# boqian-li/GarmentDreamer

Hardware: AMD Instinct MI355X
Metric: SDS iters/sec (rasterize+UNet+bwd), 100k Gaussians ×8 views @512², 1/2/4/8 GPU (higher is better)
Workload: dtype bf16

## Files before the change

### garmentdreamer_amd/csrc/nn_conv3x3.hip

```cpp
#include <hip/hip_runtime.h>
#include <stdlib.h>
#include <stdint.h>
#include <stdio.h>

#include <mutex>
#include <vector>

#include "../../include/gd_nn.h"
#include "nn_device.h"
#include "nn_host.h"

#ifndef GD_CONV_ABLATE
#define GD_CONV_ABLATE 0
#endif

namespace {

using namespace gdnn;

#ifndef GD_PATCH_EPI
#define GD_PATCH_EPI 0
#endif
typedef __attribute__((ext_vector_type(4))) float f32x4;

constexpr int BK = 64;

struct ConvGeom {
    int Hin, Win, Hg, Wg, sy, sx, Hout, Wout, osy, osx, ooy, oox, ntaps, back;
    int wtaps;
    uint64_t ty4, tx4, w4;
};

template <int BN, int BM, int WN, int WM>
__device__ __forceinline__ void conv3x3_nhwc_bf16_body(
    const uint16_t* __restrict__ in, const uint16_t* __restrict__ wt, const uint16_t* __restrict__ bias,
    int bias_img_stride, const uint16_t* __restrict__ residual, uint16_t* __restrict__ out, int Nimg, const ConvGeom& g,
    int Cin, int Cout, int tiles_n, int nwg, float* __restrict__ partial, int steps_per_split, int bid_raw, int split_idx)
{
// ... 1085 lines not shown
        g_cprof.total_flops += flops;
        g_cprof.total_bytes += bytes;
        a = b = nullptr;
    }
    ~ProfScope()
    {
        if (!a && !b) return;
        std::lock_guard<std::mutex> lk(g_cprof.mu);
        if (a) g_cprof.pool.push_back(a);
        if (b) g_cprof.pool.push_back(b);
    }
    void close_s1(int64_t M, int Cin, int Cout, bool residual)
    {
        close(2.0 * (double)M * Cout * 9.0 * Cin,
              2.0 * ((double)M * Cin + 9.0 * Cin * Cout + (double)M * Cout + (residual ? (double)M * Cout : 0.0)));
    }
};

struct TiledArgs {
    void* stream;
    const void* x;
    const float* mean_rstd;
    const void *gamma, *beta;
    int groups, silu;
    const void *w, *bias;
    int bias_img_stride;
    const void* residual;
    void* y;
    int N, H, W, Cin, Cout;
    float* stat_part;
};
constexpr int kCuLds = 160 * 1024;
static bool gn_table_fits(int lds, int Cin) { return lds + gn_table_bytes(Cin) <= kCuLds; }
template <auto Kern>
int launch_tiled(const TiledArgs& a, int lds, int tile_w, int bn, bool persistent)
{
    const int dev = current_device();
    if (dev < 0) return dev;
    if (a.mean_rstd) {
        if (!gn_table_fits(lds, a.Cin)) return fail(GD_NN_ERR_INVALID_ARG, "GroupNorm scale / shift table of Cin channels does not fit the LDS");
        lds += gn_table_bytes(a.Cin);
    }
    if (const int r = reserve_lds<Kern>(dev, a.mean_rstd ? kCuLds : lds)) return r;
    hipStream_t s = (hipStream_t)a.stream;
    const int tiles_x = (a.W + tile_w - 1) / tile_w, tiles_y = (a.H + 15) / 16, tiles_n = (a.Cout + bn - 1) / bn;
    const int nwg = a.N * tiles_x * tiles_y * tiles_n;
    int grid = nwg;
    if (persistent && nwg > num_cus(dev)) grid = (nwg & 7) == 0 ? (num_cus(dev) & ~7) : num_cus(dev);
    ProfScope prof(s);
    hipLaunchKernelGGL(Kern, dim3(grid), dim3(512), lds, s, (const uint16_t*)a.x, (const uint16_t*)a.w,
                       (const uint16_t*)a.bias, a.bias_img_stride, (const uint16_t*)a.residual, (uint16_t*)a.y, a.N, a.H,
                       a.W, a.Cin, a.Cout, a.mean_rstd, (const uint16_t*)a.gamma, (const uint16_t*)a.beta, a.groups, a.silu,
                       tiles_n, tiles_x, tiles_y, nwg, a.stat_part);
    prof.close_s1((int64_t)a.N * a.H * a.W, a.Cin, a.Cout, a.residual != nullptr);
    return launch_status();
}

}

extern "C" {

const char* gd_nn_conv_last_error(void) { return g_err; }

static int pick_split(int64_t tiles, int steps, int target = 420)
{
    int s = (int)((target + tiles / 2) / tiles);
    const int cap = steps * 2 / 15 < 24 ? steps * 2 / 15 : 24;
    if (s > cap) s = cap;
    return s < 2 ? 1 : s;
}

static size_t split_ws_bytes(int split, int64_t M, int Cout)
{
    return (size_t)split * (size_t)((M + 255) / 256 * 2) * (size_t)((Cout + 127) / 128) * 16384u * sizeof(float);
}

static int split_tile_px(int64_t M, int Cout)
{
    const int forced = conv_env().split_px;
    if (forced == 128 || forced == 256) return forced;
    M *= g_route_scale;
    return (M >= 1024 && Cout >= 1024) || M >= 2048 ? 256 : 128;
}

static bool small_tile_nosplit(int64_t M, int Cout, int ntaps, int Cin)
{
// ... 289 lines not shown
    return (size_t)((Cout + 127) / 128) * 3 * (size_t)(Cin / kWinoCK) * (size_t)kWinoWStage;
}

int gd_nn_conv3x3_wino_weights(void* stream, const void* weight, void* u, int Cout, int Cin)
{
    if (!weight || !u || Cout <= 0 || Cin <= 0) return fail(GD_NN_ERR_INVALID_ARG, "wino_weights: bad argument");
    if (Cin % kWinoCK) return fail(GD_NN_ERR_INVALID_ARG, "wino_weights: Cin % 32 != 0");
    const size_t total = gd_nn_conv3x3_wino_weights_bytes(Cout, Cin) / 16;
    const int grid = (int)((total + 255) / 256 < 4096 ? (total + 255) / 256 : 4096);
    hipLaunchKernelGGL(conv3x3_wino_weights_kernel, dim3(grid), dim3(256), 0, (hipStream_t)stream, (const uint16_t*)weight,
                       (uint16_t*)u, Cout, Cin);
    return launch_status();
}

int gd_nn_conv3x3_wino_supported(int N, int H, int W, int Cin, int Cout)
{
    if (N <= 0 || H < 16 || W < 16 || Cin <= 0 || Cout < 64) return 0;
    if (Cin % kWinoCK || Cout % 8) return 0;
    if ((double)N * H * W * Cin * 2.0 >= 2147483648.0 || (double)gd_nn_conv3x3_wino_weights_bytes(Cout, Cin) >= 2147483648.0) return 0;
    return 1;
}

static int launch_wino(void* stream, const void* x, const float* mean_rstd, const void* gamma, const void* beta, int groups,
                       int apply_silu, const void* u, const void* bias, int bias_img_stride, const void* residual, void* y,
                       int N, int H, int W, int Cin, int Cout, float* stat_part)
{
    if (!x || !u || !y) return fail(GD_NN_ERR_INVALID_ARG, "null pointer");
    if (!gd_nn_conv3x3_wino_supported(N, H, W, Cin, Cout))
        return fail(GD_NN_ERR_INVALID_ARG, "conv3x3_wino: need Cin % 32 == 0, Cout % 8 == 0, Cout >= 64, H, W >= 16, tensors < 2 GiB");
    if (mean_rstd && (!gamma || !beta || groups <= 0 || Cin % groups))
        return fail(GD_NN_ERR_INVALID_ARG, "conv3x3_wino: GroupNorm needs gamma, beta and Cin % groups == 0");
    const TiledArgs a = {stream, x, mean_rstd, gamma, beta, groups, apply_silu, u, bias, bias_img_stride, residual, y,
                         N, H, W, Cin, Cout, stat_part};
    return mean_rstd ? launch_tiled<conv3x3_wino_kernel<true>>(a, kWinoLds, 16, 128, false)
                     : launch_tiled<conv3x3_wino_kernel<false>>(a, kWinoLds, 16, 128, false);
}

int gd_nn_conv3x3_wino_forward(void* stream, const void* x, const void* u, const void* bias, int bias_img_stride,
                               const void* residual, void* y, int N, int H, int W, int Cin, int Cout, float* stat_part)
{
    return launch_wino(stream, x, nullptr, nullptr, nullptr, 0, 0, u, bias, bias_img_stride, residual, y, N, H, W, Cin,
                       Cout, stat_part);
}

int gd_nn_conv3x3_wino_gn_forward(void* stream, const void* x, const float* mean_rstd, const void* gamma, const void* beta,
                                  int groups, int apply_silu, const void* u, const void* bias, int bias_img_stride,
                                  const void* residual, void* y, int N, int H, int W, int Cin, int Cout, float* stat_part)
{
    if (!mean_rstd) return fail(GD_NN_ERR_INVALID_ARG, "conv3x3_wino_gn: mean_rstd is NULL");
    return launch_wino(stream, x, mean_rstd, gamma, beta, groups, apply_silu, u, bias, bias_img_stride, residual, y, N, H, W,
                       Cin, Cout, stat_part);
}

size_t gd_nn_conv3x3_wide_weights_bytes(int Cout, int Cin)
{
    if (Cout <= 0 || Cin <= 0 || Cin % kWideCK) return 0;
    return (size_t)((Cout + 127) / 128) * 3 * (size_t)(Cin / kWideCK) * (size_t)kWideWStage;
}

int gd_nn_conv3x3_wide_weights(void* stream, const void* weight, void* u, int Cout, int Cin)
{
    if (!weight || !u || Cout <= 0 || Cin <= 0 || Cin % kWideCK) return fail(GD_NN_ERR_INVALID_ARG, "wide_weights: bad argument");
    const size_t total = gd_nn_conv3x3_wide_weights_bytes(Cout, Cin) / 16;
    const int grid = (int)((total + 255) / 256 < 4096 ? (total + 255) / 256 : 4096);
    hipLaunchKernelGGL(conv3x3_wide_weights_kernel, dim3(grid), dim3(256), 0, (hipStream_t)stream, (const uint16_t*)weight,
                       (uint16_t*)u, Cout, Cin);
    return launch_status();
}

// ... 349 lines not shown
```

### garmentdreamer_amd/csrc/nn_conv_wino.h

```cpp
#pragma once
#include "nn_device.h"

#ifndef GD_WINO_ABLATE
#define GD_WINO_ABLATE 0
#endif

constexpr int kWinoCK = 32;
constexpr int kWinoVStage = 4 * 18 * 8 * kWinoCK * 2;
constexpr int kWinoWStage = 4 * 128 * kWinoCK * 2;
constexpr int kWinoPBytes = 21 * 1024;
constexpr int kWinoLds = 2 * kWinoVStage + 2 * kWinoWStage + kWinoPBytes;

__device__ __forceinline__ uint16_t f2bf_finite(float f)
{
    uint32_t u = __float_as_uint(f);
    u += 0x7fffu + ((u >> 16) & 1u);
    return (uint16_t)(u >> 16);
}

__global__ __launch_bounds__(256) void conv3x3_wino_weights_kernel(const uint16_t* __restrict__ w,
                                                                   uint16_t* __restrict__ u, int Cout, int Cin)
{
    const int kc = Cin / kWinoCK;
    const int tiles_n = (Cout + 127) / 128;
    const size_t total = (size_t)tiles_n * 3 * kc * 2048;
    for (size_t i = (size_t)blockIdx.x * blockDim.x + threadIdx.x; i < total; i += (size_t)gridDim.x * blockDim.x) {
        const int q = (int)(i & 2047);
        const size_t sl = i >> 11;
        const int c = (int)(sl % kc);
        const int ky = (int)((sl / kc) % 3);
        const int tn = (int)(sl / kc / 3);
        const int pc = q & 3, row = (q >> 2) & 127, pos = q >> 9;
        const int co = tn * 128 + row;
        const int ci0 = c * kWinoCK + ((pc ^ ((row >> 2) & 3)) << 3);
        uint16_t o[8];
#pragma unroll
        for (int e = 0; e < 8; e++) {
            uint16_t v = 0;
            if (co < Cout) {
                const uint16_t* g = w + ((size_t)co * 3 + ky) * 3 * Cin + ci0 + e;
                const float g0 = bf2f(g[0]), g1 = bf2f(g[Cin]), g2 = bf2f(g[2 * Cin]);
                v = pos == 0 ? g[0] : pos == 3 ? g[2 * Cin]
                    : pos == 1 ? f2bf_finite(0.5f * ((g0 + g2) + g1)) : f2bf_finite(0.5f * ((g0 + g2) - g1));
            }
            o[e] = v;
        }
        *(uint4*)(u + i * 8) = *(const uint4*)o;
    }
}

template <bool GN>
__global__ __launch_bounds__(512) void conv3x3_wino_kernel(
    const uint16_t* __restrict__ in, const uint16_t* __restrict__ uw, const uint16_t* __restrict__ bias,
    int bias_img_stride, const uint16_t* __restrict__ residual, uint16_t* __restrict__ out, int Nimg, int H, int W,
    int Cin, int Cout, const float* __restrict__ mean_rstd, const uint16_t* __restrict__ gamma,
    const uint16_t* __restrict__ beta, int G, int apply_silu, int tiles_n, int tiles_x, int tiles_y, int nwg,
    float* __restrict__ stat_part)
{
    constexpr int BN = 128;
    constexpr int THREADS = 512;
    typedef __attribute__((ext_vector_type(4))) uint32_t u32x4;
    extern __shared__ __attribute__((aligned(16))) char smem[];
    char* sV = smem;
    char* sW = smem + 2 * kWinoVStage;
    char* sP = smem + 2 * kWinoVStage + 2 * kWinoWStage;

    const int tid = threadIdx.x, lane = tid & 63;
    const int wave = __builtin_amdgcn_readfirstlane(tid >> 6);
    int bid = blockIdx.x;
    if ((nwg & 7) == 0) bid = (bid & 7) * (nwg >> 3) + (bid >> 3);
    const int tn = bid % tiles_n, tm = bid / tiles_n;
    const int tpi = tiles_x * tiles_y;
    const int nimg = tm / tpi, trem = tm - nimg * tpi;
    const int tyi = trem / tiles_x, txi = trem - tyi * tiles_x;
    const int y0 = tyi * 16 - 1, x0 = txi * 16 - 1;
    const int n0 = tn * BN;

    const uint32_t row_bytes = (uint32_t)Cin * 2u;
    const __amdgpu_buffer_rsrc_t rs_in = buffer_rsrc(in, (uint32_t)Nimg * (uint32_t)(H * W) * row_bytes);
    const int kc = Cin / kWinoCK;
    const __amdgpu_buffer_rsrc_t rs_w = buffer_rsrc(uw, (uint32_t)tiles_n * 3u * (uint32_t)kc * (uint32_t)kWinoWStage);

    uint32_t p_goff[3];
    uint32_t p_keep = 0;
#pragma unroll
    for (int i = 0; i < 3; i++) {
        const int q = tid + THREADS * i;
        const int pix = q >> 2;
        const int py = pix / kPatch, px = pix - py * kPatch;
        const int gy = y0 + py, gx = x0 + px;
        const bool inimg = pix < kPatchPix && (unsigned)gy < (unsigned)H && (unsigned)gx < (unsigned)W;
        p_goff[i] = inimg ? (uint32_t)((nimg * H + gy) * W + gx) * row_bytes + (uint32_t)(q & 3) * 16u : kOOB;
        if (inimg) p_keep |= 1u << i;
    }
    auto issueP = [&](int c) {
        if (GD_WINO_ABLATE == 3) return;
#pragma unroll
        for (int i = 0; i < 3; i++) {
            if (i == 2 && wave >= 5) continue;
            bload_lds16(rs_in, p_goff[i], (uint32_t)c * (kWinoCK * 2), sP + (wave * 64 + THREADS * i) * 16);
        }
    };
    u32x4 p_reg[3];
    auto loadP = [&](int c) {
#pragma unroll
// ... 1 lines not shown
            if (i == 2 && wave >= 5) continue;
            p_reg[i] = __builtin_bit_cast(u32x4, __builtin_amdgcn_raw_buffer_load_b128(rs_in, (int)p_goff[i],
                                                                                    (int)(c * (kWinoCK * 2)), 0));
        }
    };
    const uint32_t sP_off = (uint32_t)(uintptr_t)sP;
    const uint32_t tab_off = (uint32_t)(uintptr_t)(smem + kWinoLds);
    auto storeP = [&](int c) {
        float sc[8], sh[8];
        gn_table_read(tab_off, c * (kWinoCK / 8) + (tid & 3), sc, sh);
#pragma unroll
        for (int i = 0; i < 3; i++) {
            if (i == 2 && wave >= 5) continue;
            const bool keep = (p_keep >> i) & 1u;
            u32x4 v;
#pragma unroll
            for (int k = 0; k < 4; k++) {
                float lo = __uint_as_float(p_reg[i][k] << 16), hi = __uint_as_float(p_reg[i][k] & 0xffff0000u);
                lo = lo * sc[2 * k] + sh[2 * k];
                hi = hi * sc[2 * k + 1] + sh[2 * k + 1];
                if (apply_silu) { lo = silu_fast(lo); hi = silu_fast(hi); }
                v[k] = keep ? pack_bf16(lo, hi) : 0u;
            }
            asm volatile("ds_write_b128 %0, %1" ::"v"(sP_off + (uint32_t)(tid + THREADS * i) * 16u), "v"(v) : "memory");
        }
    };
    const uint32_t w_voff = (uint32_t)tid * 16u;
    auto issueW = [&](int buf, int ky, int c) {
        char* dst = sW + buf * kWinoWStage;
        const uint32_t soff = (uint32_t)((tn * 3 + ky) * kc + c) * (uint32_t)kWinoWStage;
#pragma unroll
        for (int i = 0; i < 4; i++)
            bload_lds16(rs_w, w_voff + (uint32_t)(THREADS * 16 * i), soff, dst + (wave * 64 + THREADS * i) * 16);
    };
    auto transform_item = [&](char* dstV, int item) {
        const int c = item & 3, t = (item >> 2) & 7, r = item >> 5;
        const char* src = sP + (r * kPatch + 2 * t) * 64 + c * 16;
        u32x4 d[4];
#pragma unroll
        for (int j = 0; j < 4; j++) d[j] = *(const u32x4*)(src + j * 64);
        uint32_t v[4][4];
#pragma unroll
        for (int k = 0; k < 4; k++) {
            const uint32_t w0 = d[0][k], w1 = d[1][k], w2 = d[2][k], w3 = d[3][k];
            const float a0 = __uint_as_float(w0 << 16), b0 = __uint_as_float(w0 & 0xffff0000u);
            const float a1 = __uint_as_float(w1 << 16), b1 = __uint_as_float(w1 & 0xffff0000u);
            const float a2 = __uint_as_float(w2 << 16), b2 = __uint_as_float(w2 & 0xffff0000u);
            const float a3 = __uint_as_float(w3 << 16), b3 = __uint_as_float(w3 & 0xffff0000u);
            v[0][k] = pack_bf16(a0 - a2, b0 - b2);
            v[1][k] = pack_bf16(a1 + a2, b1 + b2);
            v[2][k] = pack_bf16(a2 - a1, b2 - b1);
            v[3][k] = pack_bf16(a1 - a3, b1 - b3);
        }
        const int key = ((r & 1) << 1) | (t >> 2);
        const uint32_t o = (uint32_t)(uintptr_t)(dstV + r * 512 + t * 64 + ((c ^ key) << 4));
#pragma unroll
        for (int p = 0; p < 4; p++) {
            const u32x4 pv = {v[p][0], v[p][1], v[p][2], v[p][3]};
            asm volatile("ds_write_b128 %0, %1 offset:%2" ::"v"(o), "v"(pv), "n"(p * 9216) : "memory");
        }
    };

    const int pp = wave & 1, wc = (wave >> 1) & 1, wq = wave >> 2;
    const int fk = lane >> 5, fn = lane & 31;
    f32x16 acc[2][2][2];
#pragma unroll
    for (int p = 0; p < 2; p++)
#pragma unroll
        for (int a = 0; a < 2; a++)
#pragma unroll
            for (int b = 0; b < 2; b++)
#pragma unroll
                for (int k = 0; k < 16; k++) acc[p][a][b][k] = 0.f;
    uint32_t a_rd[2], b_rd[2];
#pragma unroll
    for (int a = 0; a < 2; a++) a_rd[a] = (uint32_t)((wc * 64 + a * 32 + fn) * 64);
#pragma unroll
    for (int b = 0; b < 2; b++) b_rd[b] = (uint32_t)((wq * 8 + b * 4 + (fn >> 3)) * 512 + (fn & 7) * 64);
    const uint32_t a_key = (uint32_t)((fn >> 2) & 3);
    const uint32_t b_keylo = (uint32_t)((fn & 7) >> 2);

    const int nsteps = 3 * kc;
    if (GN) {
        gn_table_fill(tab_off, tid, THREADS, Cin, G, nimg, mean_rstd, gamma, beta);
        loadP(0);
        gn_table_sync();
        storeP(0);
    } else {
        issueP(0);
    }
    issueW(0, 0, 0);
    asm volatile("s_waitcnt vmcnt(0)" ::: "memory");
    __syncthreads();
    transform_item(sV, tid);
    if (wave == 0) transform_item(sV, 512 + lane);
    __syncthreads();
    if (kc > 1) { if (GN) { loadP(1); storeP(1); } else issueP(1); }
    int s = 0;
    for (int c = 0; c < kc; c++) {
        const char* pv = sV + (c & 1) * kWinoVStage;
        char* nv = sV + ((c + 1) & 1) * kWinoVStage;
        for (int ky = 0; ky < 3; ky++, s++) {
            const int bufW = s & 1;
            asm volatile("s_waitcnt vmcnt(0)" ::: "memory");
            __syncthreads();
            if (s + 1 < nsteps && GD_WINO_ABLATE != 2) issueW(bufW ^ 1, ky == 2 ? 0 : ky + 1, ky == 2 ? c + 1 : c);
            if (c + 1 < kc) {
                if (ky == 0) {
                    if (GD_WINO_ABLATE != 1) transform_item(nv, tid);
                    if (GN && c + 2 < kc) loadP(c + 2);
                } else if (ky == 1) {
                    if (wave == (c & 7) && GD_WINO_ABLATE != 1) transform_item(nv, 512 + lane);
                } else if (c + 2 < kc) {
                    if (GN) storeP(c + 2); else issueP(c + 2);
                }
            }
            const char* pw = sW + bufW * kWinoWStage;
            const uint32_t b_key = ((((uint32_t)(fn >> 3) + (uint32_t)ky) & 1u) << 1) | b_keylo;
#pragma unroll
            for (int kk = 0; kk < 2; kk++) {
                const uint32_t ch = (uint32_t)(kk * 2 + fk);
#pragma unroll
                for (int p = 0; p < 2; p++) {
                    const int pos = 2 * pp + p;
                    bf16x8_t wf[2], vf[2];
#pragma unroll
                    for (int a = 0; a < 2; a++)
                        wf[a] = *(const bf16x8_t*)(pw + pos * (128 * 64) + a_rd[a] + ((ch ^ a_key) << 4));
#pragma unroll
                    for (int b = 0; b < 2; b++)
                        vf[b] = *(const bf16x8_t*)(pv + pos * 9216 + b_rd[b] + ky * 512 + ((ch ^ b_key) << 4));
                    if (GD_WINO_ABLATE == 4) {
#pragma unroll
                        for (int a = 0; a < 2; a++)
#pragma unroll
                            for (int b = 0; b < 2; b++) acc[p][a][b][0] += (float)wf[a][0] * (float)vf[b][1];
                    } else {
#pragma unroll
                        for (int a = 0; a < 2; a++)
#pragma unroll
                            for (int b = 0; b < 2; b++)
                                acc[p][a][b] = __builtin_amdgcn_mfma_f32_32x32x16_bf16(wf[a], vf[b], acc[p][a][b], 0, 0, 0);
                    }
                }
            }
        }
    }

    __syncthreads();
    if (GD_WINO_ABLATE != 5) {
        char* mine = smem + wave * 16384;
#pragma unroll
        for (int a = 0; a < 2; a++)
#pragma unroll
            for (int b = 0; b < 2; b++) {
#pragma unroll
                for (int q = 0; q < 4; q++) {
                    f32x4 sd;
#pragma unroll
                    for (int e = 0; e < 4; e++) sd[e] = pp ? acc[0][a][b][4 * q + e] : acc[1][a][b][4 * q + e];
                    *(f32x4*)(mine + ((a * 2 + b) * 4 + q) * 1024 + lane * 16) = sd;
                }
            }
    }
    __syncthreads();
    {
        const char* theirs = smem + (wave ^ 1) * 16384;
#pragma unroll
        for (int a = 0; a < 2; a++)
#pragma unroll
            for (int b = 0; b < 2; b++)
#pragma unroll
                for (int q = 0; q < 4; q++) {
                    const f32x4 rv = GD_WINO_ABLATE == 5 ? f32x4{0.f, 1.f, 2.f, 3.f}
                                                         : *(const f32x4*)(theirs + ((a * 2 + b) * 4 + q) * 1024 + lane * 16);
#pragma unroll
                    for (int e = 0; e < 4; e++) {
                        const float sm = acc[0][a][b][4 * q + e] + acc[1][a][b][4 * q + e];
                        acc[0][a][b][4 * q + e] = pp ? rv[e] - sm : sm + rv[e];
                    }
                }
    }
    __syncthreads();

    char* tr = smem + wave * kTrWave;
    bool ok[2];
    size_t opix[2];
#pragma unroll
    for (int b = 0; b < 2; b++) {
        const int oy = tyi * 16 + wq * 8 + b * 4 + (fn >> 3), ox = txi * 16 + 2 * (fn & 7) + pp;
        ok[b] = oy < H && ox < W;
        opix[b] = ((size_t)nimg * H + oy) * W + ox;
    }
    const uint16_t* bias_n = bias ? bias + (size_t)nimg * bias_img_stride : nullptr;
    const int stat_rows = tpi * 8;
    const int stat_row = (tyi * tiles_x + txi) * 8 + (pp * 2 + wq) * 2 + ((lane >> 4) & 1);
    const bool wide = (Cout & 7) == 0;
#pragma unroll
    for (int a = 0; a < 2; a++) {
#pragma unroll
        for (int q = 0; q < 4; q++) {
            const int co = n0 + wc * 64 + a * 32 + 8 * q + 4 * fk;
            const bool cok = co < Cout;
            float bv[4] = {0.f, 0.f, 0.f, 0.f};
            if (bias_n && cok) {
                const uint2 bb = *(const uint2*)(bias_n + co);
                bv[0] = bf2f((uint16_t)(bb.x & 0xffff)); bv[1] = bf2f((uint16_t)(bb.x >> 16));
                bv[2] = bf2f((uint16_t)(bb.y & 0xffff)); bv[3] = bf2f((uint16_t)(bb.y >> 16));
            }
            float2 st = make_float2(0.f, 0.f);
#pragma unroll
            for (int b = 0; b < 2; b++) {
                if (!ok[b] || !cok) continue;
                float v[4];
#pragma unroll
                for (int e = 0; e < 4; e++) v[e] = acc[0][a][b][4 * q + e] + bv[e];
                if (residual) {
                    const uint2 rv = *(const uint2*)(residual + opix[b] * Cout + co);
                    v[0] += bf2f((uint16_t)(rv.x & 0xffff)); v[1] += bf2f((uint16_t)(rv.x >> 16));
                    v[2] += bf2f((uint16_t)(rv.y & 0xffff)); v[3] += bf2f((uint16_t)(rv.y >> 16));
                }
                uint2 o;
                o.x = pack_bf16(v[0], v[1]);
                o.y = pack_bf16(v[2], v[3]);
                if (wide) *(uint2*)(tr + (b * 32 + fn) * kTrRow + 16 * q + 8 * fk) = o;
                else *(uint2*)(out + opix[b] * Cout + co) = o;
                if (stat_part) stat_accumulate(st, o);
            }
            if (stat_part) {
                const float sx = row16_sum(st.x), sy = row16_sum(st.y);
                if ((lane & 15) == 0 && cok)
                    *(float2*)(stat_part + (((size_t)nimg * (Cout >> 2) + (co >> 2)) * stat_rows + stat_row) * 2) =
                        make_float2(sx, sy);
            }
        }
        if (wide) {
            __builtin_amdgcn_wave_barrier();
#pragma unroll
            for (int i = 0; i < 4; i++) {
                const int pr = (lane >> 2) + 16 * i, ch = lane & 3;
                const int oy = tyi * 16 + wq * 8 + (pr >> 5) * 4 + ((pr & 31) >> 3), ox = txi * 16 + 2 * (pr & 7) + pp;
                const int co8 = n0 + wc * 64 + a * 32 + 8 * ch;
                if (oy < H && ox < W && co8 < Cout) {
                    const uint4 v = *(const uint4*)(tr + pr * kTrRow + ch * 16);
                    if (GD_WINO_ABLATE != 6 || H < 0) *(uint4*)(out + (((size_t)nimg * H + oy) * W + ox) * Cout + co8) = v;
                }
            }
            __builtin_amdgcn_wave_barrier();
        }
    }
}
```

### garmentdreamer_amd/nn_ops.py

```python
from __future__ import annotations

import ctypes as C
import os
import weakref

import torch
import torch.nn.functional as F

_HERE = os.path.dirname(os.path.abspath(__file__))
_LIB_PATH = os.path.join(_HERE, "libgd_nn.so")
_LIB_OVERRIDDEN = False
_lib = None


def use_library(path: str) -> None:
    global _LIB_PATH, _LIB_OVERRIDDEN
    if _lib is not None:
        raise RuntimeError("libgd_nn.so is already loaded")
    _LIB_PATH, _LIB_OVERRIDDEN = os.path.abspath(path), True


_vp, _i, _f = C.c_void_p, C.c_int, C.c_float
SIGNATURES = {
    "gd_nn_groupnorm_silu_forward": (_i, [_vp, _vp, _vp, _vp, _vp, _i, _i, _i, _i, _f, _i, _vp, _vp]),
# ... 2 lines not shown
    "gd_nn_groupnorm_silu_fused_forward_stats": (_i, [_vp, _vp, _vp, _vp, _vp, _i, _i, _i, _i, _f, _i, _vp]),
    "gd_nn_groupnorm_silu_fused_backward": (_i, [_vp, _vp, _vp, _vp, _vp, _vp, _vp, _i, _i, _i, _i, _i]),
    "gd_nn_groupnorm_silu_fused_backward_supported": (_i, [_i, _i, _i, _i]),
    "gd_nn_groupnorm_silu_backward": (_i, [_vp, _vp, _vp, _vp, _vp, _vp, _vp, _i, _i, _i, _i, _i, _vp, _vp, _vp]),
    "gd_nn_groupnorm_ws_bytes": (C.c_size_t, [_i, _i]),
    "gd_nn_conv3x3_forward": (_i, [_vp, _vp, _vp, _vp, _i, _vp, _vp, _i, _i, _i, _i, _i]),
    "gd_nn_conv3x3_ws_bytes": (C.c_size_t, [_i, _i, _i, _i, _i]),
    "gd_nn_conv3x3_forward_ws": (_i, [_vp, _vp, _vp, _vp, _i, _vp, _vp, _i, _i, _i, _i, _i, _vp, C.c_size_t]),
    "gd_nn_conv_force_split": (_i, [_i]),
    "gd_nn_conv_set_route_scale": (_i, [_i]),
    "gd_nn_conv3x3_flip_weights": (_i, [_vp, _vp, _vp, _i, _i]),
    "gd_nn_conv3x3_first_dgrad_supported": (_i, [_i, _i, _i, _i, _i]),
    "gd_nn_conv3x3_first_dgrad_weights": (_i, [_vp, _vp, _vp, _i, _i]),
    "gd_nn_conv3x3_first_dgrad": (_i, [_vp, _vp, _vp, _vp, _i, _i, _i, _i, _i]),
    "gd_nn_groupnorm_stats": (_i, [_vp, _vp, _i, _i, _i, _i, _f, _vp, _vp]),
    "gd_nn_groupnorm_silu_forward_fp8": (_i, [_vp, _vp, _vp, _vp, _vp, _i, _i, _i, _i, _f, _i, _vp, _vp, _f]),
    "gd_nn_conv3x3_gn_forward": (_i, [_vp, _vp, _vp, _vp, _vp, _i, _i, _vp, _vp, _i, _vp, _vp, _i, _i, _i, _i, _i]),
    "gd_nn_linear_320_supported": (_i, [C.c_int64, _i, _i]),
    "gd_nn_linear_320_forward": (_i, [_vp, _vp, _vp, _vp, _vp, C.c_int64]),
    "gd_nn_linear_k320_forward": (_i, [_vp, _vp, _vp, _vp, _vp, C.c_int64, _i]),
    "gd_nn_linear_k320_geglu_forward": (_i, [_vp, _vp, _vp, _vp, _vp, C.c_int64, _i]),
    "gd_nn_linear_320_last_error": (C.c_char_p, []),
    "gd_nn_conv3x3_stat_rows": (C.c_size_t, [_i, _i, _i, _i, _i]),
    "gd_nn_conv3x3_first_stat_rows": (C.c_size_t, [_i, _i, _i, _i, _i]),
    "gd_nn_conv3x3_first_forward_stats": (_i, [_vp, _vp, _vp, _vp, _vp, _i, _i, _i, _i, _i, _vp]),
    "gd_nn_conv3x3_gn_forward_stats": (_i, [_vp, _vp, _vp, _vp, _vp, _i, _i, _vp, _vp, _i, _vp, _vp, _i, _i, _i, _i, _i,
                                            _vp]),
    "gd_nn_conv3x3_forward_stats": (_i, [_vp, _vp, _vp, _vp, _i, _vp, _vp, _i, _i, _i, _i, _i, _vp]),
    "gd_nn_conv3x3_wino_supported": (_i, [_i, _i, _i, _i, _i]),
    "gd_nn_conv3x3_wino_weights": (_i, [_vp, _vp, _vp, _i, _i]),
    "gd_nn_conv3x3_wino_weights_bytes": (C.c_size_t, [_i, _i]),
    "gd_nn_conv3x3_wino_forward": (_i, [_vp, _vp, _vp, _vp, _i, _vp, _vp, _i, _i, _i, _i, _i, _vp]),
    "gd_nn_conv3x3_wino_gn_forward": (_i, [_vp, _vp, _vp, _vp, _vp, _i, _i, _vp, _vp, _i, _vp, _vp, _i, _i, _i, _i, _i, _vp]),
    "gd_nn_conv3x3_wide_supported": (_i, [_i, _i, _i, _i, _i]),
    "gd_nn_conv3x3_wide_weights": (_i, [_vp, _vp, _vp, _i, _i]),
    "gd_nn_conv3x3_wide_weights_bytes": (C.c_size_t, [_i, _i]),
    "gd_nn_conv3x3_wide_forward": (_i, [_vp, _vp, _vp, _vp, _i, _vp, _vp, _i, _i, _i, _i, _i, _vp]),
    "gd_nn_conv3x3_wide_gn_forward": (_i, [_vp, _vp, _vp, _vp, _vp, _i, _i, _vp, _vp, _i, _vp, _vp, _i, _i, _i, _i, _i, _vp]),
    "gd_nn_groupnorm_finish_partials": (_i, [_vp, _vp, _i, C.c_size_t, _i, _i, _i, _f, _vp]),
    "gd_nn_conv3x3_first_forward": (_i, [_vp, _vp, _vp, _vp, _vp, _i, _i, _i, _i, _i]),
    "gd_nn_conv3x3_s2_forward": (_i, [_vp, _vp, _vp, _vp, _vp, _i, _i, _i, _i, _i, _i]),
    "gd_nn_conv3x3_s2_dgrad": (_i, [_vp, _vp, _vp, _vp, _i, _i, _i, _i, _i, _i]),
    "gd_nn_conv3x3_s2_ws_bytes": (C.c_size_t, [_i, _i, _i, _i, _i, _i, _i]),
    "gd_nn_conv3x3_s2_forward_ws": (_i, [_vp, _vp, _vp, _vp, _vp, _i, _i, _i, _i, _i, _i, _vp, C.c_size_t]),
    "gd_nn_conv3x3_s2_dgrad_ws": (_i, [_vp, _vp, _vp, _vp, _i, _i, _i, _i, _i, _i, _vp, C.c_size_t]),
    "gd_nn_conv3x3_up2_forward": (_i, [_vp, _vp, _vp, _vp, _vp, _vp, _i, _i, _i, _i, _i]),
    "gd_nn_conv_force_variant": (_i, [_i]),
    "gd_nn_linear_forward": (_i, [_vp, _vp, _vp, _vp, _vp, _vp, C.c_int64, _i, _i]),
    "gd_nn_gemm_supported": (_i, [C.c_int64, _i, _i, _i]),
    "gd_nn_gemm_forward": (_i, [_vp, _vp, _vp, _vp, _vp, _vp, C.c_int64, _i, _i]),
    "gd_nn_gemm_geglu_forward": (_i, [_vp, _vp, _vp, _vp, _vp, C.c_int64, _i, _i]),
    "gd_nn_gemm_last_error": (C.c_char_p, []),
    "gd_nn_conv_profile_enable": (_i, [_i]),
    "gd_nn_conv_profile_reset": (_i, []),
    "gd_nn_conv_profile_read": (_i, [C.POINTER(C.c_double), C.POINTER(C.c_int64), C.POINTER(C.c_double)]),
    "gd_nn_conv_profile_read_bytes": (_i, [C.POINTER(C.c_double)]),
    "gd_nn_geglu_forward": (_i, [_vp, _vp, _vp, C.c_int64, _i]),
    "gd_nn_geglu_backward": (_i, [_vp, _vp, _vp, _vp, C.c_int64, _i]),
    "gd_nn_conv1x1_c8": (_i, [_vp, _vp, _vp, _vp, _vp, C.c_int64, _i]),
    "gd_nn_softmax_rows_forward": (_i, [_vp, _vp, _vp, C.c_int64, _i]),
    "gd_nn_softmax_rows_backward": (_i, [_vp, _vp, _vp, _vp, C.c_int64, _i]),
    "gd_nn_layernorm_backward": (_i, [_vp, _vp, _vp, _vp, _vp, _vp, C.c_int64, _i, C.c_float]),
    "gd_nn_add_layernorm_forward": (_i, [_vp, _vp, _vp, _vp, _vp, _f, _vp, _vp, C.c_int64, _i]),
    "gd_nn_add_layernorm_forward_bcast": (_i, [_vp, _vp, _vp, _vp, _vp, _f, _vp, _vp, C.c_int64, _i, C.c_int64]),
    "gd_nn_join_stat_rows": (C.c_size_t, [_i, _i, _i]),
    "gd_nn_add_gn_partials": (_i, [_vp, _vp, _vp, _vp, _vp, _i, _i, _i, _i]),
# ... 1965 lines not shown
```

### include/gd_nn.h

```cpp
#ifndef GD_NN_H_INCLUDED
#define GD_NN_H_INCLUDED

#include <stddef.h>
#include <stdint.h>

#ifdef __cplusplus
extern "C" {
#endif

#define GD_NN_OK 0
#define GD_NN_ERR_INVALID_ARG (-1)
#define GD_NN_ERR_HIP (-2)

int gd_nn_groupnorm_silu_forward(void* stream, const void* x, void* y, const void* gamma, const void* beta, int N,
                                 int HW, int C, int G, float eps, int apply_silu, double* stats_ws,
                                 float* mean_rstd);

int gd_nn_groupnorm_silu_backward(void* stream, const void* x, const void* dy, const void* gamma,
                                  const void* beta, const float* mean_rstd, void* dx, int N, int HW, int C, int G,
                                  int apply_silu, double* stats_ws, float* group_sums ,
                                  const void* add);

size_t gd_nn_groupnorm_ws_bytes(int N, int G);

// ... 26 lines not shown
                             const void* residual, void* y, int N, int H, int W, int Cin, int Cout, void* ws,
                             size_t ws_bytes);
int gd_nn_conv_force_split(int s);
int gd_nn_conv_set_route_scale(int k);

int gd_nn_groupnorm_silu_fused_supported(int N, int HW, int C, int G);
int gd_nn_groupnorm_silu_fused_forward(void* stream, const void* x, void* y, const void* gamma, const void* beta, int N,
                                       int HW, int C, int G, float eps, int apply_silu);
int gd_nn_groupnorm_silu_fused_forward_stats(void* stream, const void* x, void* y, const void* gamma, const void* beta, int N,
                                             int HW, int C, int G, float eps, int apply_silu, float* mean_rstd);
int gd_nn_groupnorm_silu_fused_backward_supported(int N, int HW, int C, int G);
int gd_nn_groupnorm_silu_fused_backward(void* stream, const void* x, const void* dy, const void* gamma, const void* beta,
                                        const float* mean_rstd, void* dx, int N, int HW, int C, int G, int apply_silu);

int gd_nn_groupnorm_stats(void* stream, const void* x, int N, int HW, int C, int G, float eps, double* stats_ws,
                          float* mean_rstd);

int gd_nn_conv3x3_gn_forward(void* stream, const void* x, const float* mean_rstd, const void* gamma, const void* beta,
                             int groups, int apply_silu, const void* weight, const void* bias, int bias_img_stride,
                             const void* residual, void* y, int N, int H, int W, int Cin, int Cout);

size_t gd_nn_conv3x3_stat_rows(int N, int H, int W, int Cout, int gn_entry);
int gd_nn_conv3x3_gn_forward_stats(void* stream, const void* x, const float* mean_rstd, const void* gamma,
                                   const void* beta, int groups, int apply_silu, const void* weight, const void* bias,
                                   int bias_img_stride, const void* residual, void* y, int N, int H, int W, int Cin,
                                   int Cout, float* stat_part);
int gd_nn_conv3x3_forward_stats(void* stream, const void* x, const void* weight, const void* bias, int bias_img_stride,
                                const void* residual, void* y, int N, int H, int W, int Cin, int Cout, float* stat_part);
int gd_nn_conv3x3_wino_supported(int N, int H, int W, int Cin, int Cout);
size_t gd_nn_conv3x3_wino_weights_bytes(int Cout, int Cin);
int gd_nn_conv3x3_wino_weights(void* stream, const void* weight, void* u, int Cout, int Cin);
int gd_nn_conv3x3_wino_forward(void* stream, const void* x, const void* u, const void* bias, int bias_img_stride,
                               const void* residual, void* y, int N, int H, int W, int Cin, int Cout, float* stat_part);
int gd_nn_conv3x3_wino_gn_forward(void* stream, const void* x, const float* mean_rstd, const void* gamma, const void* beta,
                                  int groups, int apply_silu, const void* u, const void* bias, int bias_img_stride,
                                  const void* residual, void* y, int N, int H, int W, int Cin, int Cout, float* stat_part);
int gd_nn_conv3x3_wide_supported(int N, int H, int W, int Cin, int Cout);
size_t gd_nn_conv3x3_wide_weights_bytes(int Cout, int Cin);
int gd_nn_conv3x3_wide_weights(void* stream, const void* weight, void* u, int Cout, int Cin);
int gd_nn_conv3x3_wide_forward(void* stream, const void* x, const void* u, const void* bias, int bias_img_stride,
                               const void* residual, void* y, int N, int H, int W, int Cin, int Cout, float* stat_part);
int gd_nn_conv3x3_wide_gn_forward(void* stream, const void* x, const float* mean_rstd, const void* gamma, const void* beta,
                                  int groups, int apply_silu, const void* u, const void* bias, int bias_img_stride,
                                  const void* residual, void* y, int N, int H, int W, int Cin, int Cout, float* stat_part);
size_t gd_nn_conv3x3_first_stat_rows(int N, int H, int W, int Cin, int Cout);
int gd_nn_conv3x3_first_forward_stats(void* stream, const void* x, const void* weight, const void* bias, void* y, int N,
                                      int H, int W, int Cin, int Cout, float* stat_part);
int gd_nn_groupnorm_finish_partials(void* stream, const float* stat_part, int N, size_t rows, int C, int G, int HW,
                                    float eps, float* mean_rstd);

int gd_nn_linear_320_supported(int64_t M, int K, int N);
int gd_nn_linear_k320_forward(void* stream, const void* x, const void* weight, const void* bias, void* y, int64_t M, int N);
int gd_nn_linear_320_forward(void* stream, const void* x, const void* weight, const void* bias, void* y, int64_t M);
int gd_nn_linear_k320_geglu_forward(void* stream, const void* x, const void* weight, const void* bias, void* y, int64_t M,
                                    int inner);
const char* gd_nn_linear_320_last_error(void);

int gd_nn_conv3x3_first_forward(void* stream, const void* x, const void* weight, const void* bias, void* y, int N, int H,
                                int W, int Cin, int Cout);

int gd_nn_conv3x3_s2_forward(void* stream, const void* x, const void* weight, const void* bias, void* y, int N, int Hin,
                             int Win, int Cin, int Cout, int pad_lo);

int gd_nn_conv3x3_up2_forward(void* stream, const void* x, const void* w_even_rows, const void* w_odd_rows,
                              const void* bias, void* y, int N, int H, int W, int Cin, int Cout);

// ... 106 lines not shown
```

Measured before the change: 22.97.

## Split Winograd conv tail tiles into half-width workgroups to balance last wave

Adds a makespan model that decides whether to split the last partial wave of 128-channel Winograd conv tiles (and any Cout tail under 64) into two 64-channel half workgroups. The kernel gains a half-tile path that loads only half the weight stage and runs one MFMA column block per wave. The aim is to cut idle CUs in the final wave of the non-GroupNorm Winograd conv. In exchange, half tiles redo the input transform, which adds redundant work and a more complex index mapping.

```diff
diff --git a/garmentdreamer_amd/csrc/nn_conv3x3.hip b/garmentdreamer_amd/csrc/nn_conv3x3.hip
--- a/garmentdreamer_amd/csrc/nn_conv3x3.hip
+++ b/garmentdreamer_amd/csrc/nn_conv3x3.hip
@@ -4,6 +4,7 @@
 #include <stdio.h>
 
 #include <mutex>
+#include <type_traits>
 #include <vector>
 
 #include "../../include/gd_nn.h"
@@ -1155,7 +1156,46 @@
 };
 constexpr int kCuLds = 160 * 1024;
 static bool gn_table_fits(int lds, int Cin) { return lds + gn_table_bytes(Cin) <= kCuLds; }
-template <auto Kern>
+
+int g_wino_halves = -1;
+int g_wino_last_halves = 0;
+constexpr double kWinoHalfCost = 0.78;
+
+double wino_makespan(int full, int halves, int cus)
+{
+    const int q = full / cus, busy = full % cus;
+    const double whole = q + (busy ? 1 : 0);
+    if (halves <= 0) return whole;
+    const auto fit = [&](double t) {
+        const int64_t na = (int64_t)((t - q) / kWinoHalfCost + 1e-6);
+        const int64_t nb = t < q + 1 ? 0 : (int64_t)((t - q - 1) / kWinoHalfCost + 1e-6);
+        return (int64_t)(cus - busy) * na + (int64_t)busy * nb >= halves;
+    };
+    for (int ka = 1, kb = 1;;) {
+        const double ta = q + ka * kWinoHalfCost, tb = q + 1 + kb * kWinoHalfCost;
+        const bool first = !busy || ta <= tb;
+        const double t = first ? ta : tb;
+        if (fit(t)) return t > whole ? t : whole;
+        if (first) ka++; else kb++;
+    }
+}
+
+int wino_plan(int m, int Cout, int cus, int* nhalf)
+{
+    const int tiles_n = (Cout + 127) / 128;
+    const bool tail = ((Cout - 1) & 127) < 64;
+    const int full = m * (tiles_n - (tail ? 1 : 0)), tails = tail ? m : 0;
+    *nhalf = 0;
+    if (g_wino_halves == 0) return m * tiles_n;
+    const int last = full % cus;
+    int r = 0;
+    if (g_wino_halves > 0) r = full;
+    else if (last && wino_makespan(full - last, tails + 2 * last, cus) < wino_makespan(full, tails, cus)) r = last;
+    *nhalf = tails + 2 * r;
+    return full - r;
+}
+
+template <auto Kern, bool Wino = false>
 int launch_tiled(const TiledArgs& a, int lds, int tile_w, int bn, bool persistent)
 {
     const int dev = current_device();
@@ -1171,10 +1211,20 @@
     int grid = nwg;
     if (persistent && nwg > num_cus(dev)) grid = (nwg & 7) == 0 ? (num_cus(dev) & ~7) : num_cus(dev);
     ProfScope prof(s);
-    hipLaunchKernelGGL(Kern, dim3(grid), dim3(512), lds, s, (const uint16_t*)a.x, (const uint16_t*)a.w,
-                       (const uint16_t*)a.bias, a.bias_img_stride, (const uint16_t*)a.residual, (uint16_t*)a.y, a.N, a.H,
-                       a.W, a.Cin, a.Cout, a.mean_rstd, (const uint16_t*)a.gamma, (const uint16_t*)a.beta, a.groups, a.silu,
-                       tiles_n, tiles_x, tiles_y, nwg, a.stat_part);
+    if constexpr (Wino) {
+        int nhalf = 0;
+        const int nfull = a.mean_rstd ? nwg : wino_plan(a.N * tiles_x * tiles_y, a.Cout, num_cus(dev), &nhalf);
+        g_wino_last_halves = nhalf;
+        hipLaunchKernelGGL(Kern, dim3(nfull + nhalf), dim3(512), lds, s, (const uint16_t*)a.x, (const uint16_t*)a.w,
+                           (const uint16_t*)a.bias, a.bias_img_stride, (const uint16_t*)a.residual, (uint16_t*)a.y, a.N,
+                           a.H, a.W, a.Cin, a.Cout, a.mean_rstd, (const uint16_t*)a.gamma, (const uint16_t*)a.beta, a.groups,
+                           a.silu, tiles_n, tiles_x, tiles_y, nwg, a.stat_part, nfull);
+    } else {
+        hipLaunchKernelGGL(Kern, dim3(grid), dim3(512), lds, s, (const uint16_t*)a.x, (const uint16_t*)a.w,
+                           (const uint16_t*)a.bias, a.bias_img_stride, (const uint16_t*)a.residual, (uint16_t*)a.y, a.N,
+                           a.H, a.W, a.Cin, a.Cout, a.mean_rstd, (const uint16_t*)a.gamma, (const uint16_t*)a.beta, a.groups,
+                           a.silu, tiles_n, tiles_x, tiles_y, nwg, a.stat_part);
+    }
     prof.close_s1((int64_t)a.N * a.H * a.W, a.Cin, a.Cout, a.residual != nullptr);
     return launch_status();
 }
@@ -1530,9 +1580,18 @@
         return fail(GD_NN_ERR_INVALID_ARG, "conv3x3_wino: GroupNorm needs gamma, beta and Cin % groups == 0");
     const TiledArgs a = {stream, x, mean_rstd, gamma, beta, groups, apply_silu, u, bias, bias_img_stride, residual, y,
                          N, H, W, Cin, Cout, stat_part};
-    return mean_rstd ? launch_tiled<conv3x3_wino_kernel<true>>(a, kWinoLds, 16, 128, false)
-                     : launch_tiled<conv3x3_wino_kernel<false>>(a, kWinoLds, 16, 128, false);
-}
+    return mean_rstd ? launch_tiled<conv3x3_wino_kernel<true>, true>(a, kWinoLds, 16, 128, false)
+                     : launch_tiled<conv3x3_wino_kernel<false>, true>(a, kWinoLds, 16, 128, false);
+}
+
+int gd_nn_conv_wino_force_halves(int mode)
+{
+    if (mode < -1 || mode > 1) return fail(GD_NN_ERR_INVALID_ARG, "wino_force_halves: mode is -1, 0 or 1");
+    g_wino_halves = mode;
+    return GD_NN_OK;
+}
+
+int gd_nn_conv_wino_last_halves(void) { return g_wino_last_halves; }
 
 int gd_nn_conv3x3_wino_forward(void* stream, const void* x, const void* u, const void* bias, int bias_img_stride,
                                const void* residual, void* y, int N, int H, int W, int Cin, int Cout, float* stat_part)
diff --git a/garmentdreamer_amd/csrc/nn_conv_wino.h b/garmentdreamer_amd/csrc/nn_conv_wino.h
--- a/garmentdreamer_amd/csrc/nn_conv_wino.h
+++ b/garmentdreamer_amd/csrc/nn_conv_wino.h
@@ -55,7 +55,7 @@
     int bias_img_stride, const uint16_t* __restrict__ residual, uint16_t* __restrict__ out, int Nimg, int H, int W,
     int Cin, int Cout, const float* __restrict__ mean_rstd, const uint16_t* __restrict__ gamma,
     const uint16_t* __restrict__ beta, int G, int apply_silu, int tiles_n, int tiles_x, int tiles_y, int nwg,
-    float* __restrict__ stat_part)
+    float* __restrict__ stat_part, int nfull)
 {
     constexpr int BN = 128;
     constexpr int THREADS = 512;
@@ -67,10 +67,37 @@
 
     const int tid = threadIdx.x, lane = tid & 63;
     const int wave = __builtin_amdgcn_readfirstlane(tid >> 6);
+    const int tpi = tiles_x * tiles_y;
     int bid = blockIdx.x;
-    if ((nwg & 7) == 0) bid = (bid & 7) * (nwg >> 3) + (bid >> 3);
-    const int tn = bid % tiles_n, tm = bid / tiles_n;
-    const int tpi = tiles_x * tiles_y;
+    int tn, tm;
+    int half = -1;
+    if (GN || nfull == nwg) {
+        if ((nwg & 7) == 0) bid = (bid & 7) * (nwg >> 3) + (bid >> 3);
+        tn = bid % tiles_n;
+        tm = bid / tiles_n;
+    } else {
+        const bool tail = ((Cout - 1) & 127) < 64;
+        const int tnf = tiles_n - (tail ? 1 : 0);
+        if (bid < nfull) {
+            if ((nfull & 7) == 0) bid = (bid & 7) * (nfull >> 3) + (bid >> 3);
+            tn = bid % tnf;
+            tm = bid / tnf;
+        } else {
+            const int nh = (int)gridDim.x - nfull, ntail = tail ? Nimg * tpi : 0;
+            int j = bid - nfull;
+            if ((nh & 7) == 0) j = (bid & 7) * (nh >> 3) + (j >> 3);
+            if (j < ntail) {
+                tn = tiles_n - 1;
+                tm = j;
+                half = 0;
+            } else {
+                const int f = nfull + ((j - ntail) >> 1);
+                tn = f % tnf;
+                tm = f / tnf;
+                half = (j - ntail) & 1;
+            }
+        }
+    }
     const int nimg = tm / tpi, trem = tm - nimg * tpi;
     const int tyi = trem / tiles_x, txi = trem - tyi * tiles_x;
     const int y0 = tyi * 16 - 1, x0 = txi * 16 - 1;
@@ -138,6 +165,16 @@
 #pragma unroll
         for (int i = 0; i < 4; i++)
             bload_lds16(rs_w, w_voff + (uint32_t)(THREADS * 16 * i), soff, dst + (wave * 64 + THREADS * i) * 16);
+    };
+    auto issueWhalf = [&](int buf, int ky, int c) {
+        char* dst = sW + buf * kWinoWStage;
+        const uint32_t soff = (uint32_t)((tn * 3 + ky) * kc + c) * (uint32_t)kWinoWStage;
+#pragma unroll
+        for (int i = 0; i < 2; i++) {
+            const int k = wave + 8 * i;
+            const int off = (k >> 2) * (128 * 64) + half * (64 * 64) + (k & 3) * 1024;
+            bload_lds16(rs_w, (uint32_t)off + (uint32_t)lane * 16u, soff, dst + off);
+        }
     };
     auto transform_item = [&](char* dstV, int item) {
         const int c = item & 3, t = (item >> 2) & 7, r = item >> 5;
@@ -167,7 +204,10 @@
         }
     };
 
-    const int pp = wave & 1, wc = (wave >> 1) & 1, wq = wave >> 2;
+    const int pp = wave & 1, wq = wave >> 2;
+    const int wc = half < 0 ? (wave >> 1) & 1 : half;
+    const int a0 = half < 0 ? 0 : (wave >> 1) & 1;
+    const int na = half < 0 ? 2 : 1;
     const int fk = lane >> 5, fn = lane & 31;
     f32x16 acc[2][2][2];
 #pragma unroll
@@ -180,7 +220,7 @@
                 for (int k = 0; k < 16; k++) acc[p][a][b][k] = 0.f;
     uint32_t a_rd[2], b_rd[2];
 #pragma unroll
-    for (int a = 0; a < 2; a++) a_rd[a] = (uint32_t)((wc * 64 + a * 32 + fn) * 64);
+    for (int a = 0; a < 2; a++) a_rd[a] = (uint32_t)((wc * 64 + (a0 + a) * 32 + fn) * 64);
 #pragma unroll
     for (int b = 0; b < 2; b++) b_rd[b] = (uint32_t)((wq * 8 + b * 4 + (fn >> 3)) * 512 + (fn & 7) * 64);
     const uint32_t a_key = (uint32_t)((fn >> 2) & 3);
@@ -195,60 +235,85 @@
     } else {
         issueP(0);
     }
-    issueW(0, 0, 0);
+    if (half < 0) issueW(0, 0, 0); else issueWhalf(0, 0, 0);
     asm volatile("s_waitcnt vmcnt(0)" ::: "memory");
     __syncthreads();
     transform_item(sV, tid);
     if (wave == 0) transform_item(sV, 512 + lane);
     __syncthreads();
     if (kc > 1) { if (GN) { loadP(1); storeP(1); } else issueP(1); }
-    int s = 0;
-    for (int c = 0; c < kc; c++) {
-        const char* pv = sV + (c & 1) * kWinoVStage;
-        char* nv = sV + ((c + 1) & 1) * kWinoVStage;
-        for (int ky = 0; ky < 3; ky++, s++) {
-            const int bufW = s & 1;
-            asm volatile("s_waitcnt vmcnt(0)" ::: "memory");
-            __syncthreads();
-            if (s + 1 < nsteps && GD_WINO_ABLATE != 2) issueW(bufW ^ 1, ky == 2 ? 0 : ky + 1, ky == 2 ? c + 1 : c);
-            if (c + 1 < kc) {
-                if (ky == 0) {
-                    if (GD_WINO_ABLATE != 1) transform_item(nv, tid);
-                    if (GN && c + 2 < kc) loadP(c + 2);
-                } else if (ky == 1) {
-                    if (wave == (c & 7) && GD_WINO_ABLATE != 1) transform_item(nv, 512 + lane);
-                } else if (c + 2 < kc) {
-                    if (GN) storeP(c + 2); else issueP(c + 2);
-                }
-            }
-            const char* pw = sW + bufW * kWinoWStage;
-            const uint32_t b_key = ((((uint32_t)(fn >> 3) + (uint32_t)ky) & 1u) << 1) | b_keylo;
-#pragma unroll
-            for (int kk = 0; kk < 2; kk++) {
-                const uint32_t ch = (uint32_t)(kk * 2 + fk);
-#pragma unroll
-                for (int p = 0; p < 2; p++) {
-                    const int pos = 2 * pp + p;
-                    bf16x8_t wf[2], vf[2];
-#pragma unroll
-                    for (int a = 0; a < 2; a++)
-                        wf[a] = *(const bf16x8_t*)(pw + pos * (128 * 64) + a_rd[a] + ((ch ^ a_key) << 4));
-#pragma unroll
-                    for (int b = 0; b < 2; b++)
-                        vf[b] = *(const bf16x8_t*)(pv + pos * 9216 + b_rd[b] + ky * 512 + ((ch ^ b_key) << 4));
-                    if (GD_WINO_ABLATE == 4) {
-#pragma unroll
-                        for (int a = 0; a < 2; a++)
-#pragma unroll
-                            for (int b = 0; b < 2; b++) acc[p][a][b][0] += (float)wf[a][0] * (float)vf[b][1];
-                    } else {
-#pragma unroll
-                        for (int a = 0; a < 2; a++)
-#pragma unroll
-                            for (int b = 0; b < 2; b++)
-                                acc[p][a][b] = __builtin_amdgcn_mfma_f32_32x32x16_bf16(wf[a], vf[b], acc[p][a][b], 0, 0, 0);
+    auto mfma_step = [&](auto blocks, const char* pw, const char* pv, int ky) {
+        constexpr int NA = decltype(blocks)::value;
+        const uint32_t b_key = ((((uint32_t)(fn >> 3) + (uint32_t)ky) & 1u) << 1) | b_keylo;
+#pragma unroll
+        for (int kk = 0; kk < 2; kk++) {
+            const uint32_t ch = (uint32_t)(kk * 2 + fk);
+#pragma unroll
+            for (int p = 0; p < 2; p++) {
+                const int pos = 2 * pp + p;
+                bf16x8_t wf[NA], vf[2];
+#pragma unroll
+                for (int a = 0; a < NA; a++)
+                    wf[a] = *(const bf16x8_t*)(pw + pos * (128 * 64) + a_rd[a] + ((ch ^ a_key) << 4));
+#pragma unroll
+                for (int b = 0; b < 2; b++)
+                    vf[b] = *(const bf16x8_t*)(pv + pos * 9216 + b_rd[b] + ky * 512 + ((ch ^ b_key) << 4));
+                if (GD_WINO_ABLATE == 4) {
+#pragma unroll
+                    for (int a = 0; a < NA; a++)
+#pragma unroll
+                        for (int b = 0; b < 2; b++) acc[p][a][b][0] += (float)wf[a][0] * (float)vf[b][1];
+                } else {
+#pragma unroll
+                    for (int a = 0; a < NA; a++)
+#pragma unroll
+                        for (int b = 0; b < 2; b++)
+                            acc[p][a][b] = __builtin_amdgcn_mfma_f32_32x32x16_bf16(wf[a], vf[b], acc[p][a][b], 0, 0, 0);
+                }
+            }
+        }
+    };
+    if (half < 0) {
+        int s = 0;
+        for (int c = 0; c < kc; c++) {
+            const char* pv = sV + (c & 1) * kWinoVStage;
+            char* nv = sV + ((c + 1) & 1) * kWinoVStage;
+#pragma unroll
+            for (int ky = 0; ky < 3; ky++, s++) {
+                const int bufW = s & 1;
+                asm volatile("s_waitcnt vmcnt(0)" ::: "memory");
+                __syncthreads();
+                if (s + 1 < nsteps && GD_WINO_ABLATE != 2) issueW(bufW ^ 1, ky == 2 ? 0 : ky + 1, ky == 2 ? c + 1 : c);
+                if (c + 1 < kc) {
+                    if (ky == 0) {
+                        if (GD_WINO_ABLATE != 1) transform_item(nv, tid);
+                        if (GN && c + 2 < kc) loadP(c + 2);
+                    } else if (ky == 1) {
+                        if (wave == (c & 7) && GD_WINO_ABLATE != 1) transform_item(nv, 512 + lane);
+                    } else if (c + 2 < kc) {
+                        if (GN) storeP(c + 2); else issueP(c + 2);
                     }
                 }
+                mfma_step(std::integral_constant<int, 2>{}, sW + bufW * kWinoWStage, pv, ky);
+            }
+        }
+    } else {
+        int s = 0;
+        for (int c = 0; c < kc; c++) {
+            const char* pv = sV + (c & 1) * kWinoVStage;
+            char* nv = sV + ((c + 1) & 1) * kWinoVStage;
+#pragma unroll
+            for (int ky = 0; ky < 3; ky++, s++) {
+                const int bufW = s & 1;
+                asm volatile("s_waitcnt vmcnt(0)" ::: "memory");
+                __syncthreads();
+                if (s + 1 < nsteps) issueWhalf(bufW ^ 1, ky == 2 ? 0 : ky + 1, ky == 2 ? c + 1 : c);
+                if (c + 1 < kc) {
+                    if (ky == 0) transform_item(nv, tid);
+                    else if (ky == 1) { if (wave == (c & 7)) transform_item(nv, 512 + lane); }
+                    else if (c + 2 < kc) issueP(c + 2);
+                }
+                mfma_step(std::integral_constant<int, 1>{}, sW + bufW * kWinoWStage, pv, ky);
             }
         }
     }
@@ -260,6 +325,7 @@
         for (int a = 0; a < 2; a++)
 #pragma unroll
             for (int b = 0; b < 2; b++) {
+                if (a >= na) continue;
 #pragma unroll
                 for (int q = 0; q < 4; q++) {
                     f32x4 sd;
@@ -278,6 +344,7 @@
             for (int b = 0; b < 2; b++)
 #pragma unroll
                 for (int q = 0; q < 4; q++) {
+                    if (a >= na) continue;
                     const f32x4 rv = GD_WINO_ABLATE == 5 ? f32x4{0.f, 1.f, 2.f, 3.f}
                                                          : *(const f32x4*)(theirs + ((a * 2 + b) * 4 + q) * 1024 + lane * 16);
 #pragma unroll
@@ -304,9 +371,10 @@
     const bool wide = (Cout & 7) == 0;
 #pragma unroll
     for (int a = 0; a < 2; a++) {
+        if (a >= na) break;
 #pragma unroll
         for (int q = 0; q < 4; q++) {
-            const int co = n0 + wc * 64 + a * 32 + 8 * q + 4 * fk;
+            const int co = n0 + wc * 64 + (a0 + a) * 32 + 8 * q + 4 * fk;
             const bool cok = co < Cout;
             float bv[4] = {0.f, 0.f, 0.f, 0.f};
             if (bias_n && cok) {
@@ -346,7 +414,7 @@
             for (int i = 0; i < 4; i++) {
                 const int pr = (lane >> 2) + 16 * i, ch = lane & 3;
                 const int oy = tyi * 16 + wq * 8 + (pr >> 5) * 4 + ((pr & 31) >> 3), ox = txi * 16 + 2 * (pr & 7) + pp;
-                const int co8 = n0 + wc * 64 + a * 32 + 8 * ch;
+                const int co8 = n0 + wc * 64 + (a0 + a) * 32 + 8 * ch;
                 if (oy < H && ox < W && co8 < Cout) {
                     const uint4 v = *(const uint4*)(tr + pr * kTrRow + ch * 16);
                     if (GD_WINO_ABLATE != 6 || H < 0) *(uint4*)(out + (((size_t)nimg * H + oy) * W + ox) * Cout + co8) = v;
diff --git a/garmentdreamer_amd/nn_ops.py b/garmentdreamer_amd/nn_ops.py
--- a/garmentdreamer_amd/nn_ops.py
+++ b/garmentdreamer_amd/nn_ops.py
@@ -58,6 +58,8 @@
     "gd_nn_conv3x3_wino_weights_bytes": (C.c_size_t, [_i, _i]),
     "gd_nn_conv3x3_wino_forward": (_i, [_vp, _vp, _vp, _vp, _i, _vp, _vp, _i, _i, _i, _i, _i, _vp]),
     "gd_nn_conv3x3_wino_gn_forward": (_i, [_vp, _vp, _vp, _vp, _vp, _i, _i, _vp, _vp, _i, _vp, _vp, _i, _i, _i, _i, _i, _vp]),
+    "gd_nn_conv_wino_force_halves": (_i, [_i]),
+    "gd_nn_conv_wino_last_halves": (_i, []),
     "gd_nn_conv3x3_wide_supported": (_i, [_i, _i, _i, _i, _i]),
     "gd_nn_conv3x3_wide_weights": (_i, [_vp, _vp, _vp, _i, _i]),
     "gd_nn_conv3x3_wide_weights_bytes": (C.c_size_t, [_i, _i]),
diff --git a/include/gd_nn.h b/include/gd_nn.h
--- a/include/gd_nn.h
+++ b/include/gd_nn.h
@@ -82,6 +82,8 @@
 int gd_nn_conv3x3_wino_weights(void* stream, const void* weight, void* u, int Cout, int Cin);
 int gd_nn_conv3x3_wino_forward(void* stream, const void* x, const void* u, const void* bias, int bias_img_stride,
                                const void* residual, void* y, int N, int H, int W, int Cin, int Cout, float* stat_part);
+int gd_nn_conv_wino_force_halves(int mode);
+int gd_nn_conv_wino_last_halves(void);
 int gd_nn_conv3x3_wino_gn_forward(void* stream, const void* x, const float* mean_rstd, const void* gamma, const void* beta,
                                   int groups, int apply_silu, const void* u, const void* bias, int bias_img_stride,
                                   const void* residual, void* y, int N, int H, int W, int Cin, int Cout, float* stat_part);
```

After: 22.98, median of 6. No clear change (+0.0%).
